# ksadov/FREUD

Measured on AMD Instinct MI355X. Metric: SAE train activations/sec (d=384 dict 8x), higher is better.
Workload: dtype bf16; 1 GPU; Whisper-tiny d=384 dict 8x (n=3072) L1 SAE train step, M=65536 rows/GPU/step, RAdam+cosine, x bfloat16 resident in HBM (BASELINE configs[1]); rows_per_gpu=65536, d_model=384, n_dict=3072, parallelism=dp1, dp=none

## Files before the change

freud_amd/csrc/bwd_fused.h:

```cpp
#pragma once
#include "common.h"
#include "gemm.h"

constexpr int BF_D = 384;
constexpr int BF_BM = 32;
constexpr int BF_BN = 128;
constexpr int BF_DXH_BYTES = BF_BM * BF_D * 2;
constexpr int BF_C_BYTES = BF_BM * BF_BN * 2;
constexpr int BF_STAGE_BYTES = 2 * BF_DXH_BYTES + BF_C_BYTES;
constexpr int BF_LDS_BYTES = 2 * BF_STAGE_BYTES;

__device__ __forceinline__ int dual_off(int row, int ch) {
  return row * 256 + ((ch ^ (((row & 3) << 2) | ((row >> 2) & 3))) << 4);
}

struct BwdFusedArgs {
  const bf16_t* dxh;
  const bf16_t* xb;
  const bf16_t* c;
  const bf16_t* Wt;
  const float* scal;
  int unscaled;
  const float* cnt_part;
  int n_cnt;
// ... 48 lines not shown
      "s_add_u32 m0, %4, %5\n\ts_nop 0\n\tglobal_load_lds_dwordx4 %2, %0 nt\n\t"
      "s_add_u32 m0, %4, %6\n\ts_nop 0\n\tglobal_load_lds_dwordx4 %3, %1 nt"
      :
      : "s"(sbase0), "s"(sbase1), "v"(voff0), "v"(voff1), "s"(base), "s"(l0), "s"(l1)
      : "memory", "m0", "scc");
}

__global__ __launch_bounds__(256, 1) void bwd_fused_d384_kernel(BwdFusedArgs a) {
  extern __shared__ __attribute__((aligned(16))) char smem[];
  const int t = threadIdx.x, lane = t & 63, w = t >> 6;
  int qa = 0, qe = 1, wgk = 0;
  unsigned long long clk_k0 = 0;
  if (a.clk) clk_k0 = __builtin_amdgcn_s_memtime();
  int wgk_raw = (int)blockIdx.x;
  if (a.bal_m > 0 && a.wg_map) wgk_raw = (int)a.wg_map[blockIdx.x];
  double cnt_m = 0;
  if (a.cnt_part) {
    for (int i0 = t; i0 < a.n_cnt; i0 += 1024) {
      float cv[4];
#pragma unroll
      for (int u = 0; u < 4; ++u) cv[u] = a.cnt_part[min(i0 + 256 * u, a.n_cnt - 1)];
#pragma unroll
      for (int u = 0; u < 4; ++u) cnt_m += i0 + 256 * u < a.n_cnt ? (double)cv[u] : 0.0;
    }
  }
  if (a.bal_m > 0) {
    wgk = __builtin_amdgcn_readfirstlane(wgk_raw);
    qa = wgk * a.bal_m;
    qe = qa + a.bal_m < 32 * a.ntiles ? qa + a.bal_m : 32 * a.ntiles;
  }
  int n0 = 0, nw = 0;
  float scal1, scal2;
  if (a.cnt_part) {
    double* redc = reinterpret_cast<double*>(smem + BF_DXH_BYTES);
    double m = wave_sum_d(cnt_m);
    if (lane == 0) redc[w] = m;
    __syncthreads();
    const double count = (double)a.M * a.d - ((redc[0] + redc[1]) + (redc[2] + redc[3]));
    scal1 = a.alpha / (float)count;
    scal2 = 1.0f / (float)a.M;
    __syncthreads();
  } else {
    scal1 = a.scal[1];
    scal2 = a.scal[2];
  }
  const float scale = a.unscaled ? scal1 : 1.0f;
  const float inv_m = a.unscaled ? scal2 / scal1 : scal2;

  const int srow = lane >> 4;
  const int pc = lane & 15;
  unsigned voff_d[6], voff_c[2];
  unsigned loff_d[6];
#pragma unroll
  for (int i = 0; i < 6; ++i) {
    const int inst = w + 4 * i, sub = inst >> 3, row = 4 * (inst & 7) + srow;
    const int ch = pc ^ (((row & 3) << 2) | ((row >> 2) & 3));
    voff_d[i] = (unsigned)(row * (BF_D * 2) + (sub * 16 + ch) * 16);
    loff_d[i] = (unsigned)__builtin_amdgcn_readfirstlane(sub * 8192 + (inst & 7) * 1024);
  }
#pragma unroll
  for (int i = 0; i < 2; ++i) {
    const int inst = w + 4 * i, row = 4 * inst + srow;
    const int ch = pc ^ (((row & 3) << 2) | ((row >> 2) & 3));
    voff_c[i] = (unsigned)(row * (a.n_p * 2) + ch * 16);
  }
  typedef __attribute__((address_space(3))) char* lptr_t;
  const unsigned smem_base = (unsigned)(uintptr_t)(lptr_t)smem;
  unsigned loff_x[6], loff_cs[2];
#pragma unroll
  for (int i = 0; i < 6; ++i) loff_x[i] = (unsigned)__builtin_amdgcn_readfirstlane((int)(loff_d[i] + 2 * BF_DXH_BYTES));
#pragma unroll
  for (int i = 0; i < 2; ++i) loff_cs[i] = (unsigned)__builtin_amdgcn_readfirstlane((w + 4 * i) * 1024);
  const unsigned stage_base_d[2] = {smem_base, smem_base + BF_DXH_BYTES};
  const unsigned stage_base_c[2] = {smem_base + 4 * BF_DXH_BYTES, smem_base + 4 * BF_DXH_BYTES + BF_C_BYTES};
  auto dma_one_at = [&](int k, const bf16_t* pd, const bf16_t* px, const bf16_t* pcl, int stage) {
    if (k < 12) {
      if ((k & 1) == 0) glds16_add(pd, voff_d[k >> 1], stage_base_d[stage], loff_d[k >> 1]);
      else glds16_add(px, voff_d[k >> 1], stage_base_d[stage], loff_x[k >> 1]);
    } else {
      glds16_add_nt(pcl, voff_c[k - 12], stage_base_c[stage], loff_cs[k - 12]);
    }
  };
  auto dma_pair_at = [&](int p, const bf16_t* pd, const bf16_t* px, const bf16_t* pcl, int stage) {
    if (p < 6) glds16_x2_add(pd, px, voff_d[p], voff_d[p], stage_base_d[stage], loff_d[p], loff_x[p]);
    else glds16_x2_add_nt(pcl, pcl, voff_c[0], voff_c[1], stage_base_c[stage], loff_cs[0], loff_cs[1]);
  };

  const int arow = lane & 31, ah = lane >> 5;
  int roff[8], toff[8];
#pragma unroll
  for (int i = 0; i < 8; ++i) roff[i] = dual_off(arow, 2 * i + ah);
  {
    const int g = (lane >> 4) & 1, q = (lane & 15) >> 2, p = lane & 3;
#pragma unroll
    for (int i = 0; i < 8; ++i) {
      const int col = 32 * (i >> 1) + 16 * g + 4 * p;
      const int r = 4 * ah + q + 8 * (i & 1);
      toff[i] = dual_off(r, col >> 3) + (col & 7) * 2;
    }
  }
  const int coff0 = [&] {
    const int g = (lane >> 4) & 1, q = (lane & 15) >> 2, p = lane & 3;
    const int col = 32 * w + 16 * g + 4 * p;
    return dual_off(4 * ah + q, col >> 3) + (col & 7) * 2;
  }();
  const int coff1 = [&] {
    const int g = (lane >> 4) & 1, q = (lane & 15) >> 2, p = lane & 3;
    const int col = 32 * w + 16 * g + 4 * p;
    return dual_off(4 * ah + q + 8, col >> 3) + (col & 7) * 2;
  }();
  int toffX[8], coffC0 = coff0 + 4 * BF_DXH_BYTES, coffC1 = coff1 + 4 * BF_DXH_BYTES;
#pragma unroll
  for (int i = 0; i < 8; ++i) {
    toffX[i] = toff[i] + 2 * BF_DXH_BYTES;
    asm volatile("" : "+v"(toffX[i]));
  }
  asm volatile("" : "+v"(coffC0), "+v"(coffC1));
  typedef __attribute__((ext_vector_type(8))) short s16x8;
  auto tr_pair = [&](const char* p0, const char* p1) -> bf16x8 {
    const s16x4 lo = __builtin_amdgcn_ds_read_tr16_b64_v4i16(LDS_PTR(s16x4, p0));
    const s16x4 hi = __builtin_amdgcn_ds_read_tr16_b64_v4i16(LDS_PTR(s16x4, p1));
    const s16x8 v = __builtin_shufflevector(lo, hi, 0, 1, 2, 3, 4, 5, 6, 7);
    return __builtin_bit_cast(bf16x8, v);
  };

  constexpr int RING = BF_RING, DIST = RING - 1;
  static_assert(72 % RING == 0, "ring slots must be static across steps");
  auto load_frag_s = [&](auto stage_tag, int i) -> bf16x8 {
    constexpr int ST = decltype(stage_tag)::value;
    if (i < 24) {
      return *reinterpret_cast<const bf16x8*>(smem + ST * BF_DXH_BYTES + (i >> 3) * 8192 + roff[i & 7]);
    } else {
      const int tt = i < 48 ? i - 24 : i - 48, dt = tt >> 1, sk = tt & 1;
      const char* b = smem + ST * BF_DXH_BYTES + (dt >> 2) * 8192 + sk * 4096;
      return i < 48 ? tr_pair(b + toff[2 * (dt & 3)], b + toff[2 * (dt & 3) + 1]) : tr_pair(b + toffX[2 * (dt & 3)], b + toffX[2 * (dt & 3) + 1]);
    }
  };
  auto load_c_s = [&](auto stage_tag, int half) -> bf16x8 {
    constexpr int ST = decltype(stage_tag)::value;
    const char* b = smem + ST * BF_C_BYTES + half * 4096;
    return tr_pair(b + coffC0, b + coffC1);
  };
  f32x16 cinit;
#pragma unroll
  for (int r = 0; r < 16; ++r) cinit[r] = inv_m;

  unsigned long long clk_t0 = 0, clk_r0 = 0, clk_loop = 0, clk_real = 0, clk_steps = 0;
#pragma unroll 1
  for (bool first_seg = true; qa < qe; first_seg = false) {
  bf16x8 wfrag[24];
  f32x16 acc[12];
  float db_acc = 0.f;
  bf16x8 ring[RING], cf[2], pf[2];
  int ntile, step_begin, step_end, split;
  if (a.bal_m > 0) {
    const int j = qa >> 5, qb = qe < 32 * (j + 1) ? qe : 32 * (j + 1);
    ntile = a.tile0 + j;
    step_begin = (qa - 32 * j) * a.bal_q;
    step_end = (qb - 32 * j) * a.bal_q;
    if (step_begin > a.steps_total) step_begin = a.steps_total;
    if (step_end > a.steps_total) step_end = a.steps_total;
    split = wgk - bal_first_wg(j, a.bal_m);
    qa = qb;
  } else {
    const int nblk = a.ntiles * a.splits;
    const int id = xcd_remap(blockIdx.x, nblk);
    split = id / a.ntiles;
    ntile = a.tile0 + id - split * a.ntiles;
    step_begin = (int)((int64_t)a.steps_total * split / a.splits);
    step_end = (int)((int64_t)a.steps_total * (split + 1) / a.splits);
    qa = qe;
  }
  ntile = __builtin_amdgcn_readfirstlane(ntile); step_begin = __builtin_amdgcn_readfirstlane(step_begin);
  step_end = __builtin_amdgcn_readfirstlane(step_end); split = __builtin_amdgcn_readfirstlane(split);
  n0 = ntile * BF_BN;
  nw = n0 + 32 * w;
  if (!first_seg) {
    asm volatile("s_waitcnt vmcnt(0) lgkmcnt(0)" ::: "memory");
    __syncthreads();
  }
  {
    const bf16_t* wp = a.Wt + (int64_t)(nw + (lane & 31)) * BF_D + 8 * (lane >> 5);
#pragma unroll
    for (int kk = 0; kk < 24; ++kk) wfrag[kk] = *reinterpret_cast<const bf16x8*>(wp + 16 * kk);
  }
#pragma unroll
  for (int i = 0; i < 12; ++i)
#pragma unroll
    for (int r = 0; r < 16; ++r) acc[i][r] = 0.f;
  db_acc = 0.f;
  if (step_begin < step_end) {
    const int64_t r0 = (int64_t)step_begin * BF_BM;
#pragma unroll
    for (int p = 0; p < 7; ++p) dma_pair_at(p, a.dxh + r0 * BF_D, a.xb + r0 * BF_D, a.c + r0 * a.n_p + n0, 0);
  }
#pragma unroll
  for (int kk = 0; kk < 24; ++kk) asm volatile("" : "+v"(wfrag[kk]));
  asm volatile("s_waitcnt vmcnt(0)" ::: "memory");
  __syncthreads();
#pragma unroll
  for (int i = 0; i <= DIST; ++i) ring[i] = load_frag_s(std::integral_constant<int, 0>{}, i);
  cf[0] = load_c_s(std::integral_constant<int, 0>{}, 0);
  cf[1] = load_c_s(std::integral_constant<int, 0>{}, 1);
  if (a.clk) { clk_t0 = __builtin_amdgcn_s_memtime(); clk_r0 = __builtin_amdgcn_s_memrealtime(); }
  const int64_t nrow_first = (int64_t)(step_begin + 1 < step_end ? step_begin + 1 : step_begin) * BF_BM;
  const bf16_t* nd = a.dxh + nrow_first * BF_D;
  const bf16_t* nx = a.xb + nrow_first * BF_D;
  const bf16_t* nc = a.c + nrow_first * a.n_p + n0;
  const int64_t c_stride = (int64_t)BF_BM * a.n_p;
  auto step_body = [&](auto cur_tag, int step) {
    constexpr int CUR = decltype(cur_tag)::value;
    using CurT = std::integral_constant<int, CUR>;
    using NxtT = std::integral_constant<int, CUR ^ 1>;
    f32x16 dc;
    bool gate_cur = false, gate_next = false;

#pragma unroll
    for (int i = 0; i < 72; ++i) {
      const bf16x8 fa = ring[i % RING];
      if (i == 0) {
        asm("v_mfma_f32_32x32x16_bf16 %0, %1, %2, %3" : "=&v"(dc) : "v"(fa), "v"(wfrag[0]), "v"(cinit));
      } else if (i < 24) {
        asm("v_mfma_f32_32x32x16_bf16 %0, %1, %2, %0" : "+v"(dc) : "v"(fa), "v"(wfrag[i]));
      } else if (i < 48) {
        acc[(i - 24) >> 1] = __builtin_amdgcn_mfma_f32_32x32x16_bf16(fa, cf[i & 1], acc[(i - 24) >> 1], 0, 0, 0);
      } else {
        acc[(i - 48) >> 1] = __builtin_amdgcn_mfma_f32_32x32x16_bf16(fa, pf[i & 1], acc[(i - 48) >> 1], 0, 0, 0);
      }
      __builtin_amdgcn_sched_barrier(0);
      const int g = i + 1;
      if (g == 72 - DIST) {
        asm volatile("s_waitcnt vmcnt(0) lgkmcnt(0)" ::: "memory");
        __builtin_amdgcn_s_barrier();
        cf[0] = load_c_s(NxtT{}, 0);
      }
      if (g == 72 - DIST + 1) cf[1] = load_c_s(NxtT{}, 1);
      if (g + DIST < 72) ring[(g + DIST) % RING] = load_frag_s(CurT{}, g + DIST);
      else ring[(g + DIST) % RING] = load_frag_s(NxtT{}, g + DIST - 72);
      if (g >= 1 && (g - 1) % 2 == 0 && (g - 1) / 2 < 14) dma_one_at((g - 1) / 2, nd, nx, nc, CUR ^ 1);
      if (g >= 29 && g < 45) {
        const int e1 = g - 29;
        gate_next = (float)cf[e1 >> 3][e1 & 7] > 0.f;
      }
      if (g >= 30 && g < 46) {
        const int e = g - 30, s2 = e >> 3, j = e & 7;
        const float gv = gate_cur ? dc[e] : 0.f;
        db_acc += gv;
        pf[s2][j] = (bf16_t)gv;
      }
      if (g >= 29 && g < 45) gate_cur = gate_next;
      __builtin_amdgcn_sched_barrier(0);
    }
    if (step + 2 < step_end) {
      nd += BF_BM * BF_D;
      nx += BF_BM * BF_D;
      nc += c_stride;
    }
  };
  {
    int step = step_begin;
    for (; step + 1 < step_end; step += 2) {
      step_body(std::integral_constant<int, 0>{}, step);
      step_body(std::integral_constant<int, 1>{}, step + 1);
    }
    if (step < step_end) step_body(std::integral_constant<int, 0>{}, step);
  }
  if (a.clk) {
    clk_loop += __builtin_amdgcn_s_memtime() - clk_t0;
    clk_real += __builtin_amdgcn_s_memrealtime() - clk_r0;
    clk_steps += (unsigned long long)(step_end - step_begin);
  }

  {
    float* out = a.slab + (int64_t)split * BF_D * a.n_p;
    const int h = lane >> 5;
    const unsigned off0 = (unsigned)(nw + (lane & 31)) + (unsigned)(4 * h) * (unsigned)a.n_p;
#pragma unroll
    for (int dt = 0; dt < 12; ++dt) {
#pragma unroll
      for (int r = 0; r < 16; ++r) {
        const unsigned drow = 32 * dt + (r & 3) + 8 * (r >> 2);
        out[off0 + drow * (unsigned)a.n_p] = acc[dt][r] * scale;
      }
      __builtin_amdgcn_sched_barrier(0);
    }
    db_acc += __shfl_xor(db_acc, 32, 64);
    if (lane < 32) a.db_part[(int64_t)split * a.n_p + nw + lane] = db_acc * scale;
  }
  }
  if (a.clk && threadIdx.x == 0) {
    unsigned long long* o = a.clk + (int64_t)blockIdx.x * 4;
    o[0] = clk_loop; o[1] = clk_real; o[2] = clk_steps; o[3] = 0;
  }
  if (a.clk && threadIdx.x == 0) {
    asm volatile("s_waitcnt vmcnt(0)" ::: "memory");
    a.clk[(int64_t)(gridDim.x + blockIdx.x) * 4] = __builtin_amdgcn_s_memtime() - clk_k0;
  }
}
```

freud_amd/csrc/common.h:

```cpp
#pragma once
#include <hip/hip_runtime.h>
#include <stdint.h>

typedef __bf16 bf16_t;
typedef __attribute__((ext_vector_type(8))) __bf16 bf16x8;
typedef __attribute__((ext_vector_type(4))) __bf16 bf16x4;
typedef __attribute__((ext_vector_type(2))) __bf16 bf16x2;
typedef __attribute__((ext_vector_type(4))) short s16x4;
typedef __attribute__((ext_vector_type(16))) float f32x16;
typedef __attribute__((ext_vector_type(4))) float f32x4;
typedef __attribute__((ext_vector_type(4))) unsigned int u32x4;

#define LDS_PTR(T, p) ((__attribute__((address_space(3))) T*)(p))

__device__ __forceinline__ float bf16_round(float v) { return (float)(bf16_t)v; }

__device__ __forceinline__ float wave_sum(float v) {
#pragma unroll
  for (int o = 32; o > 0; o >>= 1) v += __shfl_xor(v, o, 64);
  return v;
}
__device__ __forceinline__ double wave_sum_d(double v) {
#pragma unroll
  for (int o = 32; o > 0; o >>= 1) v += __shfl_xor(v, o, 64);
  return v;
}

__device__ __forceinline__ float half_wave_max_hi(float v) {
  int x = __float_as_int(v);
  x = __float_as_int(fmaxf(__int_as_float(x), __int_as_float(__builtin_amdgcn_update_dpp(x, x, 0xB1, 0xF, 0xF, false))));
  x = __float_as_int(fmaxf(__int_as_float(x), __int_as_float(__builtin_amdgcn_update_dpp(x, x, 0x4E, 0xF, 0xF, false))));
  x = __float_as_int(fmaxf(__int_as_float(x), __int_as_float(__builtin_amdgcn_update_dpp(x, x, 0x141, 0xF, 0xF, false))));
  x = __float_as_int(fmaxf(__int_as_float(x), __int_as_float(__builtin_amdgcn_update_dpp(x, x, 0x140, 0xF, 0xF, false))));
  x = __float_as_int(fmaxf(__int_as_float(x), __int_as_float(__builtin_amdgcn_update_dpp(x, x, 0x142, 0xA, 0xF, false))));
  return __int_as_float(x);
}

__device__ __forceinline__ void lds_barrier() {
  __builtin_amdgcn_sched_barrier(0);
  asm volatile("s_waitcnt lgkmcnt(0)" ::: "memory");
  __builtin_amdgcn_s_barrier();
  __builtin_amdgcn_sched_barrier(0);
}

__device__ __forceinline__ float block_sum_256_lds(float v, float* red );

__device__ __forceinline__ float block_sum_256(float v, float* red ) {
  v = wave_sum(v);
  const int w = (threadIdx.x >> 6) & 3;
  __syncthreads();
  if ((threadIdx.x & 63) == 0) red[w] = v;
  __syncthreads();
  return red[0] + red[1] + red[2] + red[3];
}
__device__ __forceinline__ float block_sum_256_lds(float v, float* red) {
  v = wave_sum(v);
  const int w = (threadIdx.x >> 6) & 3;
  lds_barrier();
  if ((threadIdx.x & 63) == 0) red[w] = v;
  lds_barrier();
  return red[0] + red[1] + red[2] + red[3];
}

__device__ __forceinline__ void glds16_x2(const void* sbase0, const void* sbase1, unsigned voff0, unsigned voff1,
                                          unsigned dst0, unsigned dst1) {
  asm volatile(
      "s_mov_b32 m0, %4\n\ts_nop 0\n\tglobal_load_lds_dwordx4 %2, %0\n\t"
      "s_mov_b32 m0, %5\n\ts_nop 0\n\tglobal_load_lds_dwordx4 %3, %1"
      :
      : "s"(sbase0), "s"(sbase1), "v"(voff0), "v"(voff1), "s"(dst0), "s"(dst1)
      : "memory", "m0");
}

__device__ __forceinline__ void glds4(const void* sbase, unsigned voff, unsigned dst) {
  asm volatile("s_mov_b32 m0, %2\n\ts_nop 0\n\tglobal_load_lds_dword %1, %0" : : "s"(sbase), "v"(voff), "s"(dst) : "memory", "m0");
}

__device__ __forceinline__ void glds16(const void* sbase, unsigned voff, unsigned dst) {
  asm volatile("s_mov_b32 m0, %2\n\ts_nop 0\n\tglobal_load_lds_dwordx4 %1, %0" : : "s"(sbase), "v"(voff), "s"(dst) : "memory", "m0");
}

#include <type_traits>
template <int B, int E, class F>
__device__ __forceinline__ void static_for(F&& f) {
  if constexpr (B < E) {
    f(std::integral_constant<int, B>{});
    static_for<B + 1, E>(f);
  }
}

static inline int64_t round_up(int64_t v, int64_t m) { return (v + m - 1) / m * m; }

__host__ __device__ __forceinline__ int bal_first_wg(int j, int m) { return (32 * j) / m; }
__host__ __device__ __forceinline__ int bal_pieces(int j, int m) { return (32 * j + 31) / m - (32 * j) / m + 1; }
```

freud_amd/csrc/engine.hip:

```cpp
#include <hip/hip_runtime.h>
#include <math.h>
#include <stdarg.h>
#include <stdio.h>
#include <string.h>

#include <algorithm>
#include <utility>
#include <vector>

#include "../../include/freud_sae.h"
#include "l1_kernels.h"
#include "gemm256.h"
#include "gemm256s.h"
#include "gemm256_fp8.h"
#include "l1_fp8.h"
#include "dp_kernels.h"
#include "p2p_exchange.h"
#include <rccl/rccl.h>
#include <mutex>
#include <unistd.h>

static thread_local bool g_force_gemm128 = false;
static thread_local bool g_no_stream = false;
static thread_local int g_device = 0;
// ... 462 lines not shown
  }
  c->slab_splits = (splits > 1 ? splits : 1) * (c->multi ? 2 : 1);
  if (c->aux_compact && c->slab_splits < 32) c->slab_splits = 32;
  TALLOC(c->slab, (int64_t)c->slab_splits * c->nW * 4);
  TALLOC(c->gn_part, 1024 * 8);
#undef TALLOC
  HIP_TRY(hipMemset(c->P, 0, c->nparams * 4));
  HIP_TRY(hipMemset(c->Mom, 0, c->nparams * 4));
  HIP_TRY(hipMemset(c->Var, 0, c->nparams * 4));
  HIP_TRY(hipMemset(c->G, 0, (c->nparams + ntail) * 4));
  HIP_TRY(hipMemset(c->nfsf, 0, (size_t)c->n_p * 8));
  int rc_ev = create_events(c);
  if (rc_ev) return rc_ev;
  HIP_TRY(hipDeviceSynchronize());
  return SAE_OK;
}

extern "C" void sae_destroy(sae_ctx* c) {
  if (!c) return;
  (void)hipSetDevice(c->cfg.device_id);
  void* ptrs[] = {c->P,    c->Mom,     c->Var,     c->G,       c->Wb,   c->Wt,      c->xb,    c->c, c->dxh, c->dxhT, c->xT,
                  c->dpre, c->slab,    c->db_part, c->l1_part, c->sq_part, c->scal, c->gn_part, c->masked, c->cn_part, c->cnt_part,
                  c->We_b, c->Wd_b, c->xs, c->pre, c->dense, c->aux_dense, c->de_b, c->dh_b, c->e, c->dh, c->e2_part,
                  c->a2_part, c->dbd_part, c->ds_part, c->tkf, c->top_idx, c->aux_idx, c->tk, c->tv_part, c->nfsf, c->dead, c->dbe_fx,
                  c->multi_dense, c->multi_idx, c->em, c->dm_b, c->m2_part, c->x8, c->c8, c->W8, c->W8t, c->scal8, c->x8_part, c->dxh8,
                  c->stats, c->stats_part, c->Gb, c->top_vals, c->aux_vals, c->multi_vals, c->tile_max, c->sel_flag, c->csc_counts, c->csc_block_off, c->csc_total, c->csc_start, c->csc_item_start,
                  c->csc_item_latent, c->csc_entries, c->csc_part, c->csc_pbe, c->tkd, c->dead_cols, c->vec_rank, c->vec_bits, c->Wdd_b,
                  c->aux_dbe_part, c->be_r, c->cnorm, c->dw_tail, c->csc_multi, c->fs_slab, c->co_zt, c->lb_lt, c->mn_w};
  for (void* p : ptrs)
    if (p) (void)hipFree(p);
  if (c->dead_hint) (void)hipHostFree(c->dead_hint);
  for (int i = 0; i < c->p2p_nopened; ++i) (void)hipIpcCloseMemHandle(c->p2p_opened[i]);
  if (c->sig) (void)hipFree(c->sig);
  if (c->p2p_status) (void)hipFree(c->p2p_status);
  if (c->p2p_status_host) (void)hipHostFree(c->p2p_status_host);
  if (c->col_stage) (void)hipFree(c->col_stage);
  if (c->bal_map) (void)hipFree(c->bal_map);
  for (void* p : {(void*)c->e32_x, (void*)c->e32_pre, (void*)c->e32_sel, (void*)c->e32_xhat, (void*)c->e32_part, (void*)c->e32_colmax})
    if (p) (void)hipFree(p);
  if (c->comm) (void)ncclCommDestroy(c->comm);
  if (c->comm_stream) (void)hipStreamDestroy(c->comm_stream);
  for (hipEvent_t e : {c->ev_x, c->ev_stats, c->ev_done})
    if (e) (void)hipEventDestroy(e);
  for (hipEvent_t e : c->ev_range)
    if (e) (void)hipEventDestroy(e);
  if (c->ev_init)
    for (auto& r : c->ev)
      for (int i = 0; i < EV_RING; ++i) {
        if (r.beg[i]) (void)hipEventDestroy(r.beg[i]);
        if (r.end[i]) (void)hipEventDestroy(r.end[i]);
      }
  delete c;
}

extern "C" int sae_create(const sae_config* cfg, sae_ctx** out) {
  if (!cfg || !out) return fail(SAE_ERR_INVALID, "null argument");
  *out = nullptr;
  if (cfg->variant != SAE_VARIANT_L1 && cfg->variant != SAE_VARIANT_TOPK)
    return fail(SAE_ERR_INVALID, "Invalid autoencoder variant: %d, must be 'l1' or 'topk'", cfg->variant);
  if (cfg->variant == SAE_VARIANT_TOPK && (cfg->k <= 0 || cfg->k > cfg->n_dict || cfg->k > 1024))
    return fail(SAE_ERR_INVALID, "topk: k=%d must be in [1, min(n_dict, 1024)]", cfg->k);
  if (cfg->variant == SAE_VARIANT_TOPK && cfg->multi_topk && (4 * cfg->k > cfg->n_dict || 4 * cfg->k > 1024))
    return fail(SAE_ERR_INVALID, "topk: multi_topk selects 4k = %d latents, must be <= min(n_dict, 1024)", 4 * cfg->k);
  if (cfg->variant != SAE_VARIANT_TOPK && cfg->multi_topk)
    return fail(SAE_ERR_INVALID, "multi_topk is a TopK option");
  if (cfg->variant == SAE_VARIANT_TOPK && cfg->d_model > 1536)
    return fail(SAE_ERR_INVALID, "topk: d_model=%d above the 1536 the sparse decoder is built for", cfg->d_model);
  if (cfg->d_model <= 0 || cfg->n_dict <= 0 || cfg->max_rows <= 0)
    return fail(SAE_ERR_INVALID, "d_model, n_dict and max_rows must be positive");
  if (cfg->optimizer != SAE_OPT_RADAM && cfg->optimizer != SAE_OPT_ADAM)
    return fail(SAE_ERR_INVALID, "Invalid optimizer: %d, must be 'radam' or 'adam'", cfg->optimizer);
  int ndev = 0;
  HIP_TRY(hipGetDeviceCount(&ndev));
  if (cfg->device_id < 0 || cfg->device_id >= ndev) return fail(SAE_ERR_INVALID, "device_id %d out of range", cfg->device_id);
  HIP_TRY(hipSetDevice(cfg->device_id));
  g_device = cfg->device_id;

  if (cfg->precision != SAE_PREC_BF16 && cfg->precision != SAE_PREC_FP8 && cfg->precision != SAE_PREC_FP8_BWD)
    return fail(SAE_ERR_INVALID, "Invalid precision: %d, must be SAE_PREC_BF16, SAE_PREC_FP8 or SAE_PREC_FP8_BWD", cfg->precision);
  if (cfg->precision != SAE_PREC_BF16 && cfg->variant != SAE_VARIANT_L1)
    return fail(SAE_ERR_INVALID, "fp8 encoder / decoder GEMMs exist for the L1 variant only");

  sae_ctx* c = new sae_ctx();
  c->cfg = *cfg;
  c->d = cfg->d_model;
  c->n = cfg->n_dict;
  c->fp8 = cfg->precision != SAE_PREC_BF16;
  c->fp8_bwd = cfg->precision == SAE_PREC_FP8_BWD;
  const int pad = c->fp8 ? 256 : 128;
  c->row_pad = pad;
  c->d_p = (int)round_up(c->d, pad);
  c->n_p = (int)round_up(c->n, pad);
  c->max_rows_p = round_up(cfg->max_rows, pad);
  c->nW = (int64_t)c->d_p * c->n_p;
  c->nparams = c->nW + c->n_p;
  c->topk = cfg->variant == SAE_VARIANT_TOPK;
  if (const char* fg = getenv("FREUD_P2P_FINEGRAINED")) c->finegrained = atoi(fg) == 1;
  const int64_t Mp = c->max_rows_p;
  if (c->topk) {
    int rc_tk = topk_create(c, Mp);
    if (rc_tk) {
      sae_destroy(c);
      return rc_tk;
    }
    *out = c;
    return SAE_OK;
  }
  g_force_gemm128 = cfg->force_gemm128 == 1;
  c->no_stream = g_no_stream = cfg->debug_flags == 86 || (getenv("FREUD_GEMM_STREAM") && atoi(getenv("FREUD_GEMM_STREAM")) == 0);
  c->dw_splits = choose_splits(c->d_p / 128, c->n_p / 128, 2 * Mp / 64);
  if (const char* ov = getenv("FREUD_DW_SPLITS")) {
    const int v = atoi(ov);
    if (v >= 1 && v <= 64) c->dw_splits = v;
  }
  c->dw_chunk_rows = c->d_p >= 1024 ? 512 : c->d_p;
  if (!g_force_gemm128 && c->d_p % 256 == 0 && c->n_p % 256 == 0 && (c->d_p / 256) * (c->n_p / 256) >= 256 && !getenv("FREUD_DW_SPLITS") &&
      c->cfg.debug_flags != 81) {
    gemm_tail_plan((c->d_p / 256) * (c->n_p / 256), (int)(2 * Mp / 64), c->dw_tail_tiles, c->dw_tail_pieces);
    if ((c->d_p / 256) * (c->n_p / 256) % 256 == 0) c->dw_tail_tiles = c->dw_tail_pieces = -1;
  }
  c->dw_chunk_splits = choose_splits(c->dw_chunk_rows / 128, c->n_p / 128, 2 * Mp / 64);
  if (c->d_p >= 1024 && c->n_p % 256 == 0)
    for (int q = 4; q >= 2; --q)
      if ((c->n_p / 256) % q == 0) {
        c->dw_col_chunks = q;
        break;
      }
  c->dw_col_splits = choose_splits(c->d_p / 128, c->n_p / 128 / c->dw_col_chunks, 2 * Mp / 64);
  c->use_fused_bwd = (c->d_p == BF_D) && cfg->force_generic != 1 && !c->fp8;
  c->use_fused_fwd = (c->d_p == FF_D) && cfg->force_generic != 1 && !c->fp8;
  if (const char* fv = getenv("FREUD_FWD")) c->fwd_variant = atoi(fv) == 1 ? 1 : 2;
  c->bwd_splits = fused_bwd_splits(c->n_p / BF_BN, (int)(Mp / BF_BM), c->n_p);
  c->bwd_range_splits = c->bwd_splits;
  for (int r = 2; r <= 4; ++r)
    if ((c->n_p / BF_BN) % r == 0) {
      const int sp = fused_bwd_splits(c->n_p / BF_BN / r, (int)(Mp / BF_BM), c->n_p / r);
      if (sp > c->bwd_range_splits) c->bwd_range_splits = sp;
    }
  int slab_splits = c->use_fused_bwd ? (c->bwd_range_splits > c->dw_splits ? c->bwd_range_splits : c->dw_splits) : c->dw_splits;
  if (c->use_fused_bwd && c->cfg.debug_flags != 83 && !getenv("FREUD_BWD_UNIFORM")) {
    const int ntiles = c->n_p / BF_BN, cus = 256;
    const int m = (32 * ntiles + cus - 1) / cus, grid = (32 * ntiles + m - 1) / m;
    int pmax = 1;
    for (int j = 0; j < ntiles; ++j) pmax = bal_pieces(j, m) > pmax ? bal_pieces(j, m) : pmax;
    const int steps = (int)(Mp / BF_BM), q = (steps + 31) / 32;
    const double slab_steps = (double)c->n_p * BF_D * 8.0 / 4.0e12 / 1.43e-6;
    const double cost_bal = (double)m * q + 5.0 + (32 % m ? 3.5 : 0.0) + (32.0 / m + (32 % m ? 1.0 : 0.0)) * slab_steps;
    const int sp = c->bwd_splits, rounds = (ntiles * sp + 255) / 256;
    const double cost_uni = rounds * ((double)((steps + sp - 1) / sp) + 5.0) + sp * slab_steps;
    if (cost_bal < cost_uni * 0.995 && pmax <= 64 && grid <= 4096) {
      c->bal_m = m;
      c->bal_grid = grid;
      if (pmax > slab_splits) slab_splits = pmax;
      std::vector<int> order(grid);
      for (int k = 0; k < grid; ++k) order[k] = k;
      std::stable_sort(order.begin(), order.end(), [m](int a_, int b_) { return (a_ * m) % 32 < (b_ * m) % 32; });
      std::vector<short> map(grid);
      int pos = 0;
      for (int x = 0; x < 8; ++x) {
        const int len = grid / 8 + (x < grid % 8 ? 1 : 0);
        for (int i = 0; i < len; ++i) map[8 * i + x] = (short)order[pos++];
      }
      hipError_t e_ = hipMalloc((void**)&c->bal_map, (size_t)grid * 2);
      if (e_ == hipSuccess) e_ = hipMemcpy(c->bal_map, map.data(), (size_t)grid * 2, hipMemcpyHostToDevice);
      if (e_ != hipSuccess) {
        int rc_ = fail(SAE_ERR_HIP, "balanced backward: workgroup table: %s", hipGetErrorString(e_));
        sae_destroy(c);
        return rc_;
      }
    }
  }
  {
    const int64_t need = (int64_t)(c->dw_chunk_splits > c->dw_col_splits ? c->dw_chunk_splits : c->dw_col_splits);
    if (need > slab_splits) slab_splits = (int)need;
  }
  const int64_t db_rows = (Mp / 128) > 64 ? (Mp / 128) : 64;

#define ALLOC(ptr, bytes)                                   \
  do {                                                      \
    hipError_t e_ = hipMalloc((void**)&(ptr), (bytes));     \
    if (e_ != hipSuccess) {                                 \
      int rc_ = fail(SAE_ERR_HIP, "hipMalloc(%lld bytes) for %s failed: %s", (long long)(bytes), #ptr, \
                     hipGetErrorString(e_));                \
      sae_destroy(c);                                       \
      return rc_;                                           \
    }                                                       \
  } while (0)
  ALLOC(c->P, c->nparams * 4);
  ALLOC(c->Mom, c->nparams * 4);
  ALLOC(c->Var, c->nparams * 4);
  if (c->finegrained) {
    hipError_t e_ = peer_visible_malloc(c, (void**)&c->G, (size_t)(c->nparams + SAE_NUM_METRICS) * 4);
    if (e_ == hipSuccess) e_ = peer_visible_malloc(c, (void**)&c->stats, (size_t)DP_STATS_HEAD * 8);
    if (e_ != hipSuccess) {
      int rc_ = fail(SAE_ERR_HIP, "fine-grained allocation of the gradient / statistics buffers failed: %s", hipGetErrorString(e_));
      sae_destroy(c);
      return rc_;
    }
  } else {
    ALLOC(c->G, (c->nparams + SAE_NUM_METRICS) * 4);
  }
  ALLOC(c->Wb, c->nW * 2);
  ALLOC(c->Wt, c->nW * 2);
  ALLOC(c->xb, Mp * c->d_p * 2);
  ALLOC(c->c, Mp * c->n_p * 2 + 4096);
  ALLOC(c->dxh, Mp * c->d_p * 2);
  ALLOC(c->dpre, Mp * c->n_p * 2);
  if (!c->use_fused_bwd && !g_force_gemm128 && c->d_p % 256 == 0 && c->n_p % 256 == 0 && Mp % 64 == 0 &&
      getenv("FREUD_DW_ROWA") && atoi(getenv("FREUD_DW_ROWA")) == 1) {
    ALLOC(c->dxhT, Mp * c->d_p * 2);
    ALLOC(c->xT, Mp * c->d_p * 2);
  }
  ALLOC(c->slab, (int64_t)slab_splits * c->nW * 4);
  ALLOC(c->db_part, db_rows * c->n_p * 4);
  ALLOC(c->l1_part, (Mp / 128) * (c->n_p / 128) * 4);
  ALLOC(c->sq_part, (Mp / 128) * (c->d_p / 128) * 2 * 4);
  ALLOC(c->scal, 16 * 4);
  ALLOC(c->gn_part, 1024 * 8);
  ALLOC(c->cn_part, (int64_t)(c->d_p / 32) * c->n_p * 4);
  ALLOC(c->cnorm, (int64_t)c->n_p * 4);
  if (c->dw_tail_tiles > 0 || (c->d_p >= 1024 && c->d_p % 256 == 0 && c->n_p % 256 == 0)) ALLOC(c->dw_tail, (int64_t)256 * 65536 * 4);
  ALLOC(c->masked, 2048 * 4);
  ALLOC(c->cnt_part, (Mp / 128 + 1) * 4);
  c->stats_cap = DP_STATS_HEAD;
  if (!c->stats) ALLOC(c->stats, c->stats_cap * 8);
  ALLOC(c->stats_part, 1024 * 4);
  if (c->fp8) {
    ALLOC(c->x8, Mp * c->d_p);
    ALLOC(c->c8, Mp * c->n_p);
    ALLOC(c->W8, c->nW);
    ALLOC(c->W8t, c->nW);
    ALLOC(c->scal8, S8_COUNT * 4);
    ALLOC(c->x8_part, 2 * 1024 * 4);
    if (c->fp8_bwd) ALLOC(c->dxh8, Mp * c->d_p);
  }
#undef ALLOC
  {
    int rc_init = [&]() -> int {
      HIP_TRY(hipMemset(c->P, 0, c->nparams * 4));
      HIP_TRY(hipMemset(c->Mom, 0, c->nparams * 4));
      HIP_TRY(hipMemset(c->Var, 0, c->nparams * 4));
      HIP_TRY(hipMemset(c->G, 0, (c->nparams + SAE_NUM_METRICS) * 4));
      int rc_ev = create_events(c);
      if (rc_ev) return rc_ev;
      HIP_TRY(hipDeviceSynchronize());
      return SAE_OK;
    }();
    if (rc_init) {
      sae_destroy(c);
      return rc_init;
    }
  }
  *out = c;
  return SAE_OK;
}

static int copy2d(void* dst, size_t dpitch, const void* src, size_t spitch, size_t width, size_t height, int to_internal,
                  int is_device) {
  hipMemcpyKind kind = is_device ? hipMemcpyDeviceToDevice : (to_internal ? hipMemcpyHostToDevice : hipMemcpyDeviceToHost);
  HIP_TRY(hipMemcpy2D(dst, dpitch, src, spitch, width, height, kind));
  return SAE_OK;
}

static int xfer_flat(sae_ctx* c, float* internal, float* w_ext, float* b_ext, int to_internal, int is_device) {
  int rc;
  if (w_ext) {
    if (to_internal)
      rc = copy2d(internal, (size_t)c->n_p * 4, w_ext, (size_t)c->n * 4, (size_t)c->n * 4, c->d, 1, is_device);
    else
      rc = copy2d(w_ext, (size_t)c->n * 4, internal, (size_t)c->n_p * 4, (size_t)c->n * 4, c->d, 0, is_device);
    if (rc) return rc;
  }
  if (b_ext) {
    hipMemcpyKind kind = is_device ? hipMemcpyDeviceToDevice : (to_internal ? hipMemcpyHostToDevice : hipMemcpyDeviceToHost);
    if (to_internal)
      HIP_TRY(hipMemcpy(internal + c->nW, b_ext, (size_t)c->n * 4, kind));
    else
      HIP_TRY(hipMemcpy(b_ext, internal + c->nW, (size_t)c->n * 4, kind));
  }
  return SAE_OK;
}

static int xfer_flat_topk(sae_ctx* c, float* internal, float* const ext[4], int to_internal, int is_device) {
  const int64_t off[4] = {0, c->nW, c->nW + c->n_p, 2 * c->nW + c->n_p};
  hipMemcpyKind kind = is_device ? hipMemcpyDeviceToDevice : (to_internal ? hipMemcpyHostToDevice : hipMemcpyDeviceToHost);
  for (int i = 0; i < 4; ++i) {
    if (!ext[i]) continue;
    float* in = internal + off[i];
    if (i == 0 || i == 2) {
      int rc = to_internal ? copy2d(in, (size_t)c->d_p * 4, ext[i], (size_t)c->d * 4, (size_t)c->d * 4, c->n, 1, is_device)
                           : copy2d(ext[i], (size_t)c->d * 4, in, (size_t)c->d_p * 4, (size_t)c->d * 4, c->n, 0, is_device);
      if (rc) return rc;
    } else {
      const size_t bytes = (size_t)(i == 1 ? c->n : c->d) * 4;
      if (to_internal) HIP_TRY(hipMemcpy(in, ext[i], bytes, kind));
      else HIP_TRY(hipMemcpy(ext[i], in, bytes, kind));
    }
  }
  return SAE_OK;
}

static void settle_weights(sae_ctx* c, hipStream_t s) {
  if (!c->wn_pending) return;
  if (c->wn_fwd_seen) {
    const int64_t n4 = c->nW / 4;
    hipLaunchKernelGGL(normalize_inplace_kernel, dim3(grid_for(n4, 2048)), dim3(256), 0, s, c->P, c->cnorm, n4, c->n_p);
  }
  c->wn_pending = c->wn_fwd_seen = false;
  c->cn_valid = false;
}

extern "C" int sae_set_params(sae_ctx* c, const float* p0, const float* p1, const float* p2, const float* p3, int is_device) {
  if (!c || !p0 || !p1) return fail(SAE_ERR_INVALID, "null argument");
  USE_DEVICE(c);
  HIP_TRY(hipDeviceSynchronize());
// ... 2566 lines not shown
```

Before: 119.1 million activations/s.

## Rotate balanced backward step walk so workgroups on one tile start at staggered rows

In the balanced fused backward kernel, each workgroup segment now starts its row walk at an offset derived from its global slot and wraps around to the start of its range. The step loop is split into runs with precomputed pointer deltas, so the wrap is handled without per-step branching. The likely aim is to spread concurrent workgroups over different rows of dxh/x/c so they hit different memory or cache lines instead of streaming the same rows at once. It adds loop-control complexity and a run-computation helper, and moves the host-side workgroup map builder into a shared header.

```diff
diff --git a/freud_amd/csrc/bwd_fused.h b/freud_amd/csrc/bwd_fused.h
--- a/freud_amd/csrc/bwd_fused.h
+++ b/freud_amd/csrc/bwd_fused.h
@@ -224,16 +224,18 @@
   f32x16 acc[12];
   float db_acc = 0.f;
   bf16x8 ring[RING], cf[2], pf[2];
-  int ntile, step_begin, step_end, split;
+  int ntile, step_begin, step_end, split, walk0;
   if (a.bal_m > 0) {
-    const int j = qa >> 5, qb = qe < 32 * (j + 1) ? qe : 32 * (j + 1);
-    ntile = a.tile0 + j;
-    step_begin = (qa - 32 * j) * a.bal_q;
-    step_end = (qb - 32 * j) * a.bal_q;
+    const BalSeg sg = bal_segment(wgk, a.bal_m, qa, qe);
+    ntile = a.tile0 + sg.tile;
+    step_begin = sg.ra * a.bal_q;
+    step_end = (sg.ra + sg.n) * a.bal_q;
+    walk0 = sg.first * a.bal_q;
     if (step_begin > a.steps_total) step_begin = a.steps_total;
     if (step_end > a.steps_total) step_end = a.steps_total;
-    split = wgk - bal_first_wg(j, a.bal_m);
-    qa = qb;
+    if (walk0 >= step_end) walk0 = step_begin;
+    split = sg.piece;
+    qa += sg.n;
   } else {
     const int nblk = a.ntiles * a.splits;
     const int id = xcd_remap(blockIdx.x, nblk);
@@ -241,10 +243,14 @@
     ntile = a.tile0 + id - split * a.ntiles;
     step_begin = (int)((int64_t)a.steps_total * split / a.splits);
     step_end = (int)((int64_t)a.steps_total * (split + 1) / a.splits);
+    walk0 = step_begin;
     qa = qe;
   }
   ntile = __builtin_amdgcn_readfirstlane(ntile); step_begin = __builtin_amdgcn_readfirstlane(step_begin);
   step_end = __builtin_amdgcn_readfirstlane(step_end); split = __builtin_amdgcn_readfirstlane(split);
+  walk0 = __builtin_amdgcn_readfirstlane(walk0);
+  const int nsteps = step_end - step_begin, wrap = step_end - walk0;
+  auto step_at = [&](int p) { return p < wrap ? walk0 + p : step_begin + p - wrap; };
   n0 = ntile * BF_BN;
   nw = n0 + 32 * w;
   if (!first_seg) {
@@ -262,7 +268,7 @@
     for (int r = 0; r < 16; ++r) acc[i][r] = 0.f;
   db_acc = 0.f;
   if (step_begin < step_end) {
-    const int64_t r0 = (int64_t)step_begin * BF_BM;
+    const int64_t r0 = (int64_t)walk0 * BF_BM;
 #pragma unroll
     for (int p = 0; p < 7; ++p) dma_pair_at(p, a.dxh + r0 * BF_D, a.xb + r0 * BF_D, a.c + r0 * a.n_p + n0, 0);
   }
@@ -275,12 +281,12 @@
   cf[0] = load_c_s(std::integral_constant<int, 0>{}, 0);
   cf[1] = load_c_s(std::integral_constant<int, 0>{}, 1);
   if (a.clk) { clk_t0 = __builtin_amdgcn_s_memtime(); clk_r0 = __builtin_amdgcn_s_memrealtime(); }
-  const int64_t nrow_first = (int64_t)(step_begin + 1 < step_end ? step_begin + 1 : step_begin) * BF_BM;
+  const int64_t nrow_first = (int64_t)step_at(1 < nsteps ? 1 : 0) * BF_BM;
   const bf16_t* nd = a.dxh + nrow_first * BF_D;
   const bf16_t* nx = a.xb + nrow_first * BF_D;
   const bf16_t* nc = a.c + nrow_first * a.n_p + n0;
-  const int64_t c_stride = (int64_t)BF_BM * a.n_p;
-  auto step_body = [&](auto cur_tag, int step) {
+  const int64_t d_bytes = (int64_t)BF_BM * BF_D * 2, c_bytes = (int64_t)BF_BM * a.n_p * 2;
+  auto step_body = [&](auto cur_tag, int64_t move_d, int64_t move_c) {
     constexpr int CUR = decltype(cur_tag)::value;
     using CurT = std::integral_constant<int, CUR>;
     using NxtT = std::integral_constant<int, CUR ^ 1>;
@@ -323,19 +329,23 @@
       if (g >= 29 && g < 45) gate_cur = gate_next;
       __builtin_amdgcn_sched_barrier(0);
     }
-    if (step + 2 < step_end) {
-      nd += BF_BM * BF_D;
-      nx += BF_BM * BF_D;
-      nc += c_stride;
-    }
+    nd = reinterpret_cast<const bf16_t*>(reinterpret_cast<const char*>(nd) + move_d);
+    nx = reinterpret_cast<const bf16_t*>(reinterpret_cast<const char*>(nx) + move_d);
+    nc = reinterpret_cast<const bf16_t*>(reinterpret_cast<const char*>(nc) + move_c);
   };
   {
-    int step = step_begin;
-    for (; step + 1 < step_end; step += 2) {
-      step_body(std::integral_constant<int, 0>{}, step);
-      step_body(std::integral_constant<int, 1>{}, step + 1);
-    }
-    if (step < step_end) step_body(std::integral_constant<int, 0>{}, step);
+    int step = 0;
+#pragma unroll 1
+    while (step + 1 < nsteps) {
+      const BalRun run = bal_run(step, nsteps, wrap);
+      const int run_hi = __builtin_amdgcn_readfirstlane(run.hi);
+      const int64_t ed = run.d_even * d_bytes, ec = run.d_even * c_bytes, od = run.d_odd * d_bytes, oc = run.d_odd * c_bytes;
+      for (; step < run_hi; step += 2) {
+        step_body(std::integral_constant<int, 0>{}, ed, ec);
+        step_body(std::integral_constant<int, 1>{}, od, oc);
+      }
+    }
+    if (step < nsteps) step_body(std::integral_constant<int, 0>{}, 0, 0);
   }
   if (a.clk) {
     clk_loop += __builtin_amdgcn_s_memtime() - clk_t0;
diff --git a/freud_amd/csrc/bwd_walk.h b/freud_amd/csrc/bwd_walk.h
--- /dev/null
+++ b/freud_amd/csrc/bwd_walk.h
@@ -0,0 +1,69 @@
+#pragma once
+#include <algorithm>
+#include <vector>
+
+#if defined(__HIPCC__)
+#define BW_HD __host__ __device__ __forceinline__
+#else
+#define BW_HD inline
+#endif
+
+BW_HD int bal_first_wg(int j, int m) { return (32 * j) / m; }
+BW_HD int bal_pieces(int j, int m) { return (32 * j + 31) / m - (32 * j) / m + 1; }
+
+struct BalSeg {
+  int tile;
+  int ra, n;
+  int slot0;
+  int piece;
+  int first;
+};
+
+BW_HD BalSeg bal_segment(int k, int m, int qa, int qe) {
+  BalSeg s;
+  s.tile = qa >> 5;
+  const int qb = qe < 32 * (s.tile + 1) ? qe : 32 * (s.tile + 1);
+  s.ra = qa - 32 * s.tile;
+  s.n = qb - qa;
+  s.slot0 = qa - k * m;
+  s.piece = k - bal_first_wg(s.tile, m);
+  int d = (s.slot0 - s.ra) % m;
+  if (d < 0) d += m;
+  s.first = d < s.n ? s.ra + d : s.ra;
+  return s;
+}
+
+BW_HD int bal_move(int p, int nsteps, int wrap) { return p + 2 >= nsteps ? 0 : (p + 2 == wrap ? 1 - nsteps : 1); }
+
+struct BalRun {
+  int hi, d_even, d_odd;
+};
+BW_HD BalRun bal_run(int pos, int nsteps, int wrap) {
+  const int none = 0x7fffffff;
+  const int e1 = (wrap >= 2 && wrap < nsteps) ? ((wrap - 2) & ~1) : none;
+  const int e2 = (nsteps - 2) & ~1;
+  BalRun r;
+  r.d_even = bal_move(pos, nsteps, wrap);
+  r.d_odd = bal_move(pos + 1, nsteps, wrap);
+  if (pos == e1 || pos == e2) {
+    r.hi = pos + 2;
+  } else {
+    r.hi = nsteps & ~1;
+    if (e1 > pos && e1 < r.hi) r.hi = e1;
+    if (e2 > pos && e2 < r.hi) r.hi = e2;
+  }
+  return r;
+}
+
+inline std::vector<short> bal_build_map(int m, int grid) {
+  std::vector<int> order(grid);
+  for (int k = 0; k < grid; ++k) order[k] = k;
+  std::stable_sort(order.begin(), order.end(), [m](int a, int b) { return (a * m) % 32 < (b * m) % 32; });
+  std::vector<short> map(grid);
+  int pos = 0;
+  for (int x = 0; x < 8; ++x) {
+    const int len = grid / 8 + (x < grid % 8 ? 1 : 0);
+    for (int i = 0; i < len; ++i) map[8 * i + x] = (short)order[pos++];
+  }
+  return map;
+}
diff --git a/freud_amd/csrc/common.h b/freud_amd/csrc/common.h
--- a/freud_amd/csrc/common.h
+++ b/freud_amd/csrc/common.h
@@ -91,5 +91,4 @@
 
 static inline int64_t round_up(int64_t v, int64_t m) { return (v + m - 1) / m * m; }
 
-__host__ __device__ __forceinline__ int bal_first_wg(int j, int m) { return (32 * j) / m; }
-__host__ __device__ __forceinline__ int bal_pieces(int j, int m) { return (32 * j + 31) / m - (32 * j) / m + 1; }
+#include "bwd_walk.h"
diff --git a/freud_amd/csrc/engine.hip b/freud_amd/csrc/engine.hip
--- a/freud_amd/csrc/engine.hip
+++ b/freud_amd/csrc/engine.hip
@@ -638,15 +638,7 @@
       c->bal_m = m;
       c->bal_grid = grid;
       if (pmax > slab_splits) slab_splits = pmax;
-      std::vector<int> order(grid);
-      for (int k = 0; k < grid; ++k) order[k] = k;
-      std::stable_sort(order.begin(), order.end(), [m](int a_, int b_) { return (a_ * m) % 32 < (b_ * m) % 32; });
-      std::vector<short> map(grid);
-      int pos = 0;
-      for (int x = 0; x < 8; ++x) {
-        const int len = grid / 8 + (x < grid % 8 ? 1 : 0);
-        for (int i = 0; i < len; ++i) map[8 * i + x] = (short)order[pos++];
-      }
+      const std::vector<short> map = bal_build_map(m, grid);
       hipError_t e_ = hipMalloc((void**)&c->bal_map, (size_t)grid * 2);
       if (e_ == hipSuccess) e_ = hipMemcpy(c->bal_map, map.data(), (size_t)grid * 2, hipMemcpyHostToDevice);
       if (e_ != hipSuccess) {
```

Result: no change. 119.4 million activations/s, median of 6 (+0.3%).
